# qdLMF/LightGlue-with-FlashAttentionV2-TensorRT

Hardware: AMD Instinct MI355X
Metric: attention-calls/sec & ms/call, 1×1024×1024 d=64 fp16; % MFMA peak (higher is better)
Workload: dtype fp16; 1 GPU; MHAHeadDim64 plugin enqueue, Q/K/V [1,4,1024,64] fp16 -> O fp16 (BASELINE configs[1]); K independent plugin enqueues per timed repetition; batch=1, heads=4, nq=1024, nkv=1024, head_dim=64, parallelism=replicas1, pairs=one pair stream per GPU, no collective

## Files before the change

lightglue-with-flashattentionv2-tensorrt_amd/csrc/lightglue_ffn.hip:

```cpp
#include <stdlib.h>

#include <atomic>
#include <cstdlib>

#include "lightglue_device.h"

namespace {

#ifdef LG_LN_STAMPS
__device__ unsigned long long g_ln_stamps[256 * 8 * 8];
#define LN_SEG(k)                                                                                    \
    do {                                                                                             \
        unsigned long long t_;                                                                       \
        asm volatile("s_waitcnt lgkmcnt(0)\n\ts_memtime %0\n\ts_waitcnt lgkmcnt(0)" : "=s"(t_)::"memory"); \
        sg_[k] += t_ - last_;                                                                        \
        last_ = t_;                                                                                  \
    } while (0)
#else
#define LN_SEG(k) \
    do {          \
    } while (0)
#endif
constexpr int kLnN = 512;
template <int KS, int MT, int BK, int NST, int NWV = 8>
// ... 71 lines not shown
        for (int ks = 0; ks < KS; ++ks) {
            const int gs = t * KS + ks;
            if (ks == 0 && t == 0) LN_SEG(0);
            else LN_SEG(2);
            if (gs + NST - 2 > nsteps - 1) asm volatile("s_waitcnt vmcnt(0) lgkmcnt(0)" ::: "memory");
            else if (ks < NST - 1 && t > 0) asm volatile("s_waitcnt vmcnt(%0) lgkmcnt(0)" ::"n"((NST - 2) * D + SPW) : "memory");
            else asm volatile("s_waitcnt vmcnt(%0) lgkmcnt(0)" ::"n"((NST - 2) * D) : "memory");
            __builtin_amdgcn_s_barrier();
            LN_SEG(1);
            {
                char* const fb = smem + (st == 0 ? NST - 1 : st - 1) * SB;
                if (ks + NST - 1 < KS) tile_issue<true, BK, KS, NT, NWV>(cur, ks + NST - 1, fb, wave);
                else if (more) tile_issue<true, BK, KS, NT, NWV>(src_of(t + 1), ks + NST - 1 - KS, fb, wave);
            }
            const unsigned sb = (unsigned)(st * SB);
            st_last = st;
            st = st == NST - 1 ? 0 : st + 1;
#pragma unroll
            for (int s = 0; s < BK / 16; ++s) {
                const int u = 2 * s + hh;
                f16x8 wf[NB], af[2];
#pragma unroll
                for (int b = 0; b < NB; ++b) wf[b] = *(lds_f16x8*)(lds + sb + wro[b] + ((u ^ wsw[b]) << 4));
#pragma unroll
                for (int b = 0; b < 2; ++b) af[b] = *(lds_f16x8*)(lds + sb + aro[b] + ((u ^ asw[b]) << 4));
#pragma unroll
                for (int nb = 0; nb < NB; ++nb)
#pragma unroll
                    for (int mb = 0; mb < 2; ++mb)
                        acc[nb][mb] = __builtin_amdgcn_mfma_f32_32x32x16_f16(wf[nb], af[mb], acc[nb][mb], 0, 0, 0);
            }
        }

        LN_SEG(2);
        const int nw0 = wn * WTN;
        float rs[2];
#pragma unroll
        for (int mb = 0; mb < 2; ++mb) {
            float s = 0.f;
#pragma unroll
            for (int nb = 0; nb < NB; ++nb)
#pragma unroll
                for (int g = 0; g < 4; ++g) {
                    const u32x2 b4 = *(__attribute__((address_space(3))) u32x2*)(lds + kPar + (nw0 + 32 * nb + 8 * g + 4 * hh) * 2);
#pragma unroll
                    for (int u = 0; u < 4; ++u) {
                        const float a = acc[nb][mb][4 * g + u];
                        const float h = (u & 1) ? mixh<1>(a, b4[u >> 1]) : mixh<0>(a, b4[u >> 1]);
                        acc[nb][mb][4 * g + u] = h;
                        s += h;
                    }
                }
            rs[mb] = s + __shfl_xor(s, 32, 64);
        }
        if (hh == 0) {
#pragma unroll
            for (int mb = 0; mb < 2; ++mb) red[(wm * 64 + 32 * mb + r) * WN + wn] = rs[mb];
        }
        asm volatile("s_waitcnt lgkmcnt(0)" ::: "memory");
        __builtin_amdgcn_s_barrier();
        float mean[2];
#pragma unroll
        for (int mb = 0; mb < 2; ++mb) {
            mean[mb] = red_sum((wm * 64 + 32 * mb + r) * WN) * (1.f / kLnN);
            float q = 0.f;
#pragma unroll
            for (int nb = 0; nb < NB; ++nb)
#pragma unroll
                for (int e = 0; e < 16; ++e) {
                    const float d = acc[nb][mb][e] - mean[mb];
                    acc[nb][mb][e] = d;
                    q = __builtin_fmaf(d, d, q);
                }
            rs[mb] = q + __shfl_xor(q, 32, 64);
        }
        if (hh == 0) {
#pragma unroll
            for (int mb = 0; mb < 2; ++mb) red[MT * WN + (wm * 64 + 32 * mb + r) * WN + wn] = rs[mb];
        }
        asm volatile("s_waitcnt lgkmcnt(0)" ::: "memory");
        __builtin_amdgcn_s_barrier();
        LN_SEG(3);
        lds_char* const stg = lds + st_last * SB + wave * 4096;
#pragma unroll
        for (int mb = 0; mb < 2; ++mb) {
            const float rstd = __builtin_amdgcn_rsqf(red_sum(MT * WN + (wm * 64 + 32 * mb + r) * WN) * (1.f / kLnN) + eps);
#pragma unroll
            for (int np = 0; np < NP; ++np) {
#pragma unroll
                for (int nbl = 0; nbl < 2; ++nbl)
#pragma unroll
                    for (int g = 0; g < 4; ++g) {
                        const int n = nw0 + 64 * np + 32 * nbl + 8 * g + 4 * hh;
                        const u32x2 g4 = *(__attribute__((address_space(3))) u32x2*)(lds + kPar + NT * 2 + n * 2);
                        const u32x2 b4 = *(__attribute__((address_space(3))) u32x2*)(lds + kPar + 2 * NT * 2 + n * 2);
                        f16x4 o;
#pragma unroll
                        for (int u = 0; u < 4; u += 2) {
                            const f32x16& av = acc[2 * np + nbl][mb];
                            const f32x2 xr = f32x2{av[4 * g + u], av[4 * g + u + 1]} * rstd;
                            const f32x2 gl = gelu_as2(f32x2{mixf<0>(xr[0], g4[u >> 1], b4[u >> 1]), mixf<1>(xr[1], g4[u >> 1], b4[u >> 1])});
                            o[u] = (f16)gl[0];
                            o[u + 1] = (f16)gl[1];
                        }
                        *(__attribute__((address_space(3))) f16x4*)(stg + r * 128 + (((4 * nbl + g) ^ (r & 7)) << 4) + 8 * hh) = o;
                    }
                f16x8 o8[4];
#pragma unroll
                for (int i = 0; i < 4; ++i) {
                    const int rl = 8 * i + cr;
                    o8[i] = *(lds_f16x8*)(stg + rl * 128 + ((cc ^ (rl & 7)) << 4));
                }
#pragma unroll
                for (int i = 0; i < 4; ++i) {
                    const int row = min(m0 + wm * 64 + 32 * mb + 8 * i + cr, p.m - 1);
                    st_out(p.out[0] + (size_t)row * NT + nw0 + 64 * np + 8 * cc, o8[i]);
                }
            }
        }
        if (more) cur = src_of(t + 1);
    }
    asm volatile("s_waitcnt vmcnt(0)" ::: "memory");
    LN_SEG(4);
#ifdef LG_LN_STAMPS
    if (lane == 0) {
        unsigned long long* d = g_ln_stamps + ((size_t)blockIdx.x * 8 + wave) * 8;
        for (int k = 0; k < 5; ++k) d[k] = sg_[k];
        d[5] = last_ - t_entry_;
        d[6] = (unsigned long long)ntile_w;
    }
#endif
}


constexpr int kFfnOut = 256;

enum { E3_NONE = 0, E3_SPLIT2 = 1, E3_QKV = 2, E3_PLAIN = 3 };
struct Proj3 {
    const f16* b3;
    const f16* cosv;
    const f16* sinv;
    f16* out[6];
    int n_store;
};
#ifdef LG_FR_STAMPS
__device__ unsigned long long g_fr_stamps[256 * 8 * 8];
#define FR_SEG(k)                                                                                    \
    do {                                                                                             \
        unsigned long long t_;                                                                       \
        asm volatile("s_waitcnt lgkmcnt(0)\n\ts_memtime %0\n\ts_waitcnt lgkmcnt(0)" : "=s"(t_)::"memory"); \
        fr_[k] = t_ - fr_last_;                                                                      \
        fr_last_ = t_;                                                                               \
    } while (0)
#else
#define FR_SEG(k) \
    do {          \
    } while (0)
#endif
__device__ __forceinline__ void row_dev2(unsigned h2, float c, f32x2& q) {
    const f32x2 d = f32x2{mixn<0>(h2, 1.f, -c), mixn<1>(h2, 1.f, -c)};
    q = d * d + q;
}
struct RowStats {
    float mean, rstd;
};
__device__ __forceinline__ RowStats ln_merge(f32x4 sa, f32x4 sc, f32x4 qa, f32x4 qc, float eps) {
    const float mean = (((sa[0] + sa[1]) + (sa[2] + sa[3])) + ((sc[0] + sc[1]) + (sc[2] + sc[3]))) * (1.f / 512);
    const f32x4 da = sa * (1.f / 64) - mean, dc = sc * (1.f / 64) - mean;
    const f32x4 ba = da * da, bc = dc * dc;
    const float within = ((qa[0] + qa[1]) + (qa[2] + qa[3])) + ((qc[0] + qc[1]) + (qc[2] + qc[3]));
    const float between = ((ba[0] + ba[1]) + (ba[2] + ba[3])) + ((bc[0] + bc[1]) + (bc[2] + bc[3]));
    return {mean, __builtin_amdgcn_rsqf(fmaf(between, 64.f, within) * (1.f / 512) + eps)};
}
template <int MB, int D, int E3, int NB3>
__global__ __launch_bounds__(512, 1) void ffn_rows_kernel(LinArgs p, const f16* __restrict__ gamma,
                                                          const f16* __restrict__ beta, float eps,
                                                          const f16* __restrict__ wp, const f16* __restrict__ b2,
                                                          Proj3 q3) {
    constexpr int MT = 32 * MB;
    constexpr int K = 512, NO = kFfnOut;
    constexpr int kA = 0, kH = MT * K * 2;
    constexpr int kSP = 80;
    constexpr int kStg = MB == 1 ? 2 * kH : kH;
    constexpr int kPar = MB == 1 ? kStg + 8 * MT * kSP : 2 * kH;
    constexpr int kRed = kPar + (3 * K + NO) * 2;
    constexpr int NS1 = K / 16, NS = 2 * NS1;
    constexpr int NS3 = NO / 16;
    constexpr int NP = 96 + NB3 * NS3;
    constexpr int R = 2 * D;
    static_assert(D >= 1 && D <= NS1 && (MB == 1 || MB == 2) && (E3 == E3_NONE) == (NB3 == 0), "shape");
    static_assert(MB == 1 || 8 * MT * kSP <= kH, "staging over h");
    constexpr int kB3 = kRed + 2 * MT * 8 * 4;
    constexpr int kCS = kB3 + NB3 * 256 * 2;
    constexpr int kCSP = 144;
    constexpr int kEnd = kCS + (E3 == E3_QKV ? 2 * MT * kCSP : 0);
    static_assert(kEnd <= 160 * 1024, "LDS");
    __shared__ __attribute__((aligned(16))) char smem[kEnd];
    lds_char* const lds = (lds_char*)smem;
    const int tid = threadIdx.x, lane = tid & 63;
    const int wave = __builtin_amdgcn_readfirstlane(tid >> 6);
    const int r = lane & 31, hh = lane >> 5;
    const int m0 = blockIdx.x * MT;
#ifdef LG_FR_STAMPS
    unsigned long long fr_[6] = {0, 0, 0, 0, 0, 0}, fr_last_, fr_entry_;
    asm volatile("s_memtime %0\n\ts_waitcnt lgkmcnt(0)" : "=s"(fr_entry_)::"memory");
    fr_last_ = fr_entry_;
#endif

    constexpr bool AH = MB == 1;
    f16x8 av[AH ? 1 : 4 * MB], ax[2 * MB], ac[2 * MB];
    if constexpr (AH) {
#pragma unroll
        for (int i = 0; i < 2 * MB; ++i) {
            const int grow = min(m0 + 16 * i + 2 * wave + (lane >> 5), p.m - 1);
            ax[i] = *reinterpret_cast<const f16x8*>(p.a + (size_t)grow * (K / 2) + (lane & 31) * 8);
        }
#pragma unroll
        for (int i = 0; i < 2 * MB; ++i) {
            const int grow = min(m0 + 16 * i + 2 * wave + (lane >> 5), p.m - 1);
            const LinRow lr = lin_row(p, grow, (lane & 31) >> 3);
            ac[i] = *reinterpret_cast<const f16x8*>((lr.first ? p.ctx0 : p.ctx1) + lr.off + (lane & 7) * 8);
        }
    } else {
#pragma unroll
        for (int i = 0; i < 4 * MB; ++i) {
            const int grow = min(m0 + 8 * i + wave, p.m - 1);
            const f16* src;
            if (lane < 32) {
                src = p.a + (size_t)grow * (K / 2) + lane * 8;
            } else {
                const LinRow lr = lin_row(p, grow, (lane - 32) >> 3);
                src = (lr.first ? p.ctx0 : p.ctx1) + lr.off + ((lane - 32) & 7) * 8;
            }
            av[i] = *reinterpret_cast<const f16x8*>(src);
        }
    }
    f16x8 pv = {};
    if (tid < 224) {
        const f16* const pvs = tid < 64 ? p.bias : tid < 128 ? gamma : tid < 192 ? beta : b2;
        pv = *reinterpret_cast<const f16x8*>(pvs + (tid & 63) * 8);
    }

    constexpr int NV3 = NB3 * 256 * 2 / 16 + (E3 == E3_QKV ? 2 * MT * kD * 2 / 16 : 0);
    constexpr int NV3T = (NV3 + 511) / 512;
    f16x8 v3[NV3T > 0 ? NV3T : 1];
#pragma unroll
    for (int i = 0; i < NV3T; ++i) {
        const int u = i * 512 + tid;
        if (u < NB3 * 256 * 2 / 16) {
            v3[i] = *reinterpret_cast<const f16x8*>(q3.b3 + u * 8);
        } else if (u < NV3) {
            const int cu = u - NB3 * 256 * 2 / 16, t = cu / (MT * 8), rw = min(m0 + (cu % (MT * 8)) / 8, p.m - 1);
            v3[i] = *reinterpret_cast<const f16x8*>((t ? q3.sinv : q3.cosv) + (size_t)rw * kD + (cu % 8) * 8);
        }
    }

    asm volatile("s_barrier" ::: "memory");

    const __amdgpu_buffer_rsrc_t wrs = __builtin_amdgcn_make_buffer_rsrc(const_cast<f16*>(wp), (short)0, 8 * NP * 1024, 0x00020000);
    const unsigned wo = (unsigned)(wave * NP * 1024 + lane * 16);
    auto piece = [&](int i) { return __builtin_bit_cast(f16x8, __builtin_amdgcn_raw_buffer_load_b128(wrs, wo, i * 1024, 0)); };
    f16x8 q[R];
#pragma unroll
    for (int i = 0; i < R; ++i) {
        q[i] = piece(i);
        if (i & 1) __builtin_amdgcn_sched_barrier(0);
    }
    auto take = [&](int i) {
        const f16x8 w = q[i % R];
        if (i + R < NP) q[i % R] = piece(i + R);
        return w;
    };
    auto put_half = [&](const f16x8 (&hv)[2 * MB], int u0) {
#pragma unroll
        for (int i = 0; i < 2 * MB; ++i) {
            const int row = 16 * i + 2 * wave + (lane >> 5), u = u0 + (lane & 31);
            *(lds_f16x8*)(lds + kA + row * 1024 + ((u ^ (row & 15)) << 4)) = hv[i];
        }
    };
    if constexpr (AH) {
        put_half(ax, 0);
    } else {
#pragma unroll
        for (int i = 0; i < 4 * MB; ++i) {
            const int row = 8 * i + wave;
            *(lds_f16x8*)(lds + kA + row * 1024 + ((lane ^ (row & 15)) << 4)) = av[i];
        }
    }
    if (tid < 224) *(lds_f16x8*)(lds + kPar + tid * 16) = pv;
#pragma unroll
    for (int i = 0; i < NV3T; ++i)
        if (i * 512 + tid < NB3 * 256 * 2 / 16) {
            *(lds_f16x8*)(lds + kB3 + (i * 512 + tid) * 16) = v3[i];
        } else if (i * 512 + tid < NV3) {
            const int cu = i * 512 + tid - NB3 * 256 * 2 / 16;
            *(lds_f16x8*)(lds + kCS + (cu / 8) * kCSP + (cu % 8) * 16) = v3[i];
        }
    asm volatile("s_waitcnt lgkmcnt(0)" ::: "memory");
    __builtin_amdgcn_s_barrier();
    FR_SEG(0);

    struct BF {
        f16x8 v[MB];
    };
    auto bfrag = [&](int base, int s) {
        BF f;
#pragma unroll
        for (int mb = 0; mb < MB; ++mb) {
// ... 109 lines not shown
        asm volatile("s_waitcnt lgkmcnt(0)" ::: "memory");
        __builtin_amdgcn_s_barrier();
    }

    lds_char* const stg = lds + kStg + wave * (MT * kSP);
#pragma unroll
    for (int mb = 0; mb < MB; ++mb)
#pragma unroll
        for (int g = 0; g < 4; ++g) {
            const int c = 32 * wave + 8 * g + 4 * hh;
            const f16x4 b4 = *(__attribute__((address_space(3))) f16x4*)(lds + kPar + 3 * K * 2 + c * 2);
            const f16x4 v = f16x4{lin_val(o2[mb][4 * g], b4[0]), lin_val(o2[mb][4 * g + 1], b4[1]),
                                  lin_val(o2[mb][4 * g + 2], b4[2]), lin_val(o2[mb][4 * g + 3], b4[3])};
            *(__attribute__((address_space(3))) f16x4*)(stg + (32 * mb + r) * kSP + (8 * g + 4 * hh) * 2) = v;
        }
    asm volatile("s_waitcnt lgkmcnt(0)" ::: "memory");
    f16x8 xo[MB][2];
#pragma unroll
    for (int mb = 0; mb < MB; ++mb) {
        const int rr = 32 * mb + (lane >> 1), half = lane & 1;
#pragma unroll
        for (int e2 = 0; e2 < 2; ++e2) {
            f16x8 v = *(lds_f16x8*)(stg + rr * kSP + half * 32 + e2 * 16);
            const f16x8 xr = *(lds_f16x8*)(lds + kA + rr * 1024 + (((4 * wave + 2 * half + e2) ^ (rr & 15)) << 4));
#pragma unroll
            for (int e = 0; e < 8; ++e) v[e] = res_add(v[e], xr[e]);
            xo[mb][e2] = v;
            if (m0 + rr < p.m) *reinterpret_cast<f16x8*>(p.out[0] + (size_t)(m0 + rr) * NO + 32 * wave + 16 * half + 8 * e2) = v;
        }
    }
#ifdef LG_FR_STAMPS
    asm volatile("s_waitcnt vmcnt(0)" ::: "memory");
    FR_SEG(4);
#endif
    if constexpr (E3 != E3_NONE) {
        asm volatile("s_waitcnt lgkmcnt(0)" ::: "memory");
        __builtin_amdgcn_s_barrier();
#pragma unroll
        for (int mb = 0; mb < MB; ++mb) {
            const int rr = 32 * mb + (lane >> 1), half = lane & 1;
#pragma unroll
            for (int e2 = 0; e2 < 2; ++e2)
                *(lds_f16x8*)(lds + kA + rr * 512 + (((4 * wave + 2 * half + e2) ^ (rr & 15)) << 4)) = xo[mb][e2];
        }
        asm volatile("s_waitcnt lgkmcnt(0)" ::: "memory");
        __builtin_amdgcn_s_barrier();
        auto xfrag = [&](int s) {
            BF f;
#pragma unroll
            for (int mb = 0; mb < MB; ++mb) {
                const int row = 32 * mb + r;
                f.v[mb] = *(lds_f16x8*)(lds + kA + row * 512 + (((2 * s + hh) ^ (row & 15)) << 4));
            }
            return f;
        };
        f32x16 a3[NB3][MB] = {};
        BF xf = xfrag(0);
#pragma unroll
        for (int j = 0; j < NS3; ++j) {
            f16x8 w3[NB3];
#pragma unroll
            for (int b = 0; b < NB3; ++b) w3[b] = take(96 + NB3 * j + b);
            const BF xn = j + 1 < NS3 ? xfrag(j + 1) : xf;
#pragma unroll
            for (int b = 0; b < NB3; ++b)
#pragma unroll
                for (int mb = 0; mb < MB; ++mb) a3[b][mb] = __builtin_amdgcn_mfma_f32_32x32x16_f16(w3[b], xf.v[mb], a3[b][mb], 0, 0, 0);
            xf = xn;
            __builtin_amdgcn_sched_barrier(0);
        }
#pragma unroll
        for (int b = 0; b < NB3; ++b) {
            const int cb = 32 * (NB3 * wave + b);
#pragma unroll
            for (int mb = 0; mb < MB; ++mb)
#pragma unroll
                for (int g = 0; g < 4; ++g) {
                    const int c = cb + 8 * g + 4 * hh;
                    const f16x4 b4 = *(__attribute__((address_space(3))) f16x4*)(lds + kB3 + c * 2);
                    f16x4 v = f16x4{lin_val(a3[b][mb][4 * g], b4[0]), lin_val(a3[b][mb][4 * g + 1], b4[1]),
                                    lin_val(a3[b][mb][4 * g + 2], b4[2]), lin_val(a3[b][mb][4 * g + 3], b4[3])};
                    if constexpr (E3 == E3_QKV) {
                        if (cb < 2 * NO) {
                            const int rw = 32 * mb + r;
                            const f16x4 cc = *(__attribute__((address_space(3))) f16x4*)(lds + kCS + rw * kCSP + (c % kD) * 2);
                            const f16x4 ss = *(__attribute__((address_space(3))) f16x4*)(lds + kCS + (MT + rw) * kCSP + (c % kD) * 2);
#pragma unroll
                            for (int t = 0; t < 4; t += 2) rot_pair(v, t, cc[t], ss[t], cc[t + 1], ss[t + 1]);
                        }
                    }
                    *(__attribute__((address_space(3))) f16x4*)(stg + (32 * mb + r) * kSP + (8 * g + 4 * hh) * 2) = v;
                }
            asm volatile("s_waitcnt lgkmcnt(0)" ::: "memory");
#pragma unroll
            for (int mb = 0; mb < MB; ++mb) {
                const int rr = 32 * mb + (lane >> 1), half = lane & 1;
                const f16x8 v0 = *(lds_f16x8*)(stg + rr * kSP + half * 32);
                const f16x8 v1 = *(lds_f16x8*)(stg + rr * kSP + half * 32 + 16);
                const int row = m0 + rr;
                if (row < p.m) {
                    f16* dst;
                    if constexpr (E3 == E3_PLAIN) {
                        dst = cb < q3.n_store ? q3.out[0] + (size_t)row * q3.n_store + cb + 16 * half : nullptr;
                    } else {
                        const int part = cb / NO, h = (cb % NO) / kD;
                        const LinRow lr = lin_row(p, row, h);
                        dst = q3.out[E3 == E3_QKV ? (lr.first ? 0 : 3) + part : (lr.first ? 0 : 1) + 2 * part] + lr.off +
                              cb % kD + 16 * half;
                    }
                    if (dst) {
                        *reinterpret_cast<f16x8*>(dst) = v0;
                        *reinterpret_cast<f16x8*>(dst + 8) = v1;
                    }
                }
            }
            asm volatile("s_waitcnt lgkmcnt(0)" ::: "memory");
        }
    }
#ifdef LG_FR_STAMPS
    asm volatile("s_waitcnt vmcnt(0)" ::: "memory");
    FR_SEG(5);
    if (lane == 0 && blockIdx.x < 256) {
        unsigned long long* d = g_fr_stamps + ((size_t)blockIdx.x * 8 + wave) * 8;
        for (int k = 0; k < 5; ++k) d[k] = fr_[k];
        d[5] = fr_last_ - fr_entry_;
        d[6] = fr_entry_;
        d[7] = fr_[5];
    }
#endif
}

template <int D, int E3, int NB3, int SP = 1>
__global__ __launch_bounds__(512, 1) void ffn_rows16_kernel(LinArgs p, const f16* __restrict__ gamma,
                                                            const f16* __restrict__ beta, float eps,
                                                            const f16* __restrict__ wp, const f16* __restrict__ b2,
                                                            Proj3 q3) {
    constexpr int MT = 16, K = 512, NO = kFfnOut;
    constexpr int NP = 96 + NB3 * 16;
    constexpr int R = 2 * D;
    constexpr int NB = 2 * NB3;
    constexpr int NBP = NB / (SP > 1 ? SP : 1);
    constexpr int NPS = 96 + 8 * NBP;
    constexpr int U3 = 32 * NB3;
    constexpr int kA = 0;
    constexpr int kH = kA + MT * 1024;
    constexpr int kX = kH + MT * 1024;
    constexpr int kS3 = kX + MT * 512;
    constexpr int kPar = kS3 + MT * U3 * 16;
    constexpr int kRed = kPar + (3 * K + NO) * 2;
    constexpr int kB3 = kRed + 2 * MT * 8 * 4;
    constexpr int kCS = kB3 + NB3 * 256 * 2;
    constexpr int kCSP = 144;
    constexpr int kEnd = kCS + (E3 == E3_QKV ? 2 * MT * kCSP : 0);
    static_assert(D >= 1 && D <= 16 && (E3 == E3_NONE) == (NB3 == 0) && kEnd <= 160 * 1024, "shape");
    static_assert(SP == 1 || (E3 != E3_NONE && NB % SP == 0), "parts");
    __shared__ __attribute__((aligned(16))) char smem[kEnd];
    lds_char* const lds = (lds_char*)smem;
    const int tid = threadIdx.x, lane = tid & 63;
    const int wave = __builtin_amdgcn_readfirstlane(tid >> 6);
    const int r = lane & 15, q = lane >> 4;
    const int part = SP > 1 ? (int)blockIdx.x % SP : 0;
    const int m0 = (SP > 1 ? (int)blockIdx.x / SP : (int)blockIdx.x) * MT;
#ifdef LG_FR_STAMPS
    unsigned long long fr_[7] = {0, 0, 0, 0, 0, 0, 0}, fr_last_, fr_entry_;
    asm volatile("s_memtime %0\n\ts_waitcnt lgkmcnt(0)" : "=s"(fr_entry_)::"memory");
    fr_last_ = fr_entry_;
#endif
    auto tile_unit = [](int row, int u) { return row * 1024 + ((u ^ (row & 15)) << 4); };
    auto x_unit = [](int row, int u) { return row * 512 + ((u ^ (row & 15)) << 4); };

    f16x8 ax, ac;
    {
        const int grow = min(m0 + (tid >> 5), p.m - 1);
        ax = *reinterpret_cast<const f16x8*>(p.a + (size_t)grow * (K / 2) + (tid & 31) * 8);
        const LinRow lr = lin_row(p, grow, (tid & 31) >> 3);
        ac = *reinterpret_cast<const f16x8*>((lr.first ? p.ctx0 : p.ctx1) + lr.off + (tid & 7) * 8);
    }
    f16x8 pv = {};
    if (tid < 224) {
        const f16* const pvs = tid < 64 ? p.bias : tid < 128 ? gamma : tid < 192 ? beta : b2;
        pv = *reinterpret_cast<const f16x8*>(pvs + (tid & 63) * 8);
    }
    constexpr int NVB = NB3 * 256 * 2 / 16;
    constexpr int NV3 = NVB + (E3 == E3_QKV ? 2 * MT * 8 : 0);
    static_assert(NV3 <= 512, "phase 3 vectors");
    f16x8 v3 = {};
    if (tid < NV3) {
        if (tid < NVB) {
            v3 = *reinterpret_cast<const f16x8*>(q3.b3 + tid * 8);
        } else {
            const int cu = tid - NVB, t = cu / (MT * 8), rw = min(m0 + (cu % (MT * 8)) / 8, p.m - 1);
            v3 = *reinterpret_cast<const f16x8*>((t ? q3.sinv : q3.cosv) + (size_t)rw * kD + (cu % 8) * 8);
        }
    }
    asm volatile("s_barrier" ::: "memory");

    const __amdgpu_buffer_rsrc_t wrs = __builtin_amdgcn_make_buffer_rsrc(const_cast<f16*>(wp), (short)0, 8 * NP * 1024, 0x00020000);
    const unsigned wo = (unsigned)(wave * NP * 1024 + lane * 16);
    const int p3off = __builtin_amdgcn_readfirstlane(part * NBP * 1024);
    auto piece = [&](int i) {
        const int so = i < 96 ? i * 1024 : (96 + NB * ((i - 96) / NBP) + (i - 96) % NBP) * 1024 + p3off;
        return __builtin_bit_cast(f16x8, __builtin_amdgcn_raw_buffer_load_b128(wrs, wo, so, 0));
    };
    f16x8 w_[R];
#pragma unroll
    for (int i = 0; i < R; ++i) {
        w_[i] = piece(i);
        if (i & 1) __builtin_amdgcn_sched_barrier(0);
    }
    auto take = [&](int i) {
        const f16x8 w = w_[i % R];
        if (i + R < NPS) w_[i % R] = piece(i + R);
        return w;
    };
    *(lds_f16x8*)(lds + kA + tile_unit(tid >> 5, tid & 31)) = ax;
    if (tid < 224) *(lds_f16x8*)(lds + kPar + tid * 16) = pv;
    if (tid < NVB) {
        *(lds_f16x8*)(lds + kB3 + tid * 16) = v3;
    } else if (tid < NV3) {
        const int cu = tid - NVB;
        *(lds_f16x8*)(lds + kCS + (cu / 8) * kCSP + (cu % 8) * 16) = v3;
    }
    asm volatile("s_waitcnt lgkmcnt(0)" ::: "memory");
    __builtin_amdgcn_s_barrier();
    FR_SEG(0);

    f32x4 acc[4] = {};
    f16x8 bf = *(lds_f16x8*)(lds + kA + tile_unit(r, q));
#pragma unroll
    for (int s = 0; s < 16; ++s) {
        f16x8 w4[4];
#pragma unroll
        for (int b = 0; b < 4; ++b) w4[b] = take(4 * s + b);
        if (s + 1 == 8) {
            *(lds_f16x8*)(lds + kA + tile_unit(tid >> 5, 32 + (tid & 31))) = ac;
            asm volatile("s_waitcnt lgkmcnt(0)" ::: "memory");
            __builtin_amdgcn_s_barrier();
        }
        const f16x8 bn = s + 1 < 16 ? *(lds_f16x8*)(lds + kA + tile_unit(r, 4 * (s + 1) + q)) : bf;
#pragma unroll
        for (int b = 0; b < 4; ++b) acc[b] = __builtin_amdgcn_mfma_f32_16x16x32_f16(w4[b], bf, acc[b], 0, 0, 0);
        bf = bn;
        __builtin_amdgcn_sched_barrier(0);
    }
    FR_SEG(1);

    float* const red = (float*)(void*)(smem + kRed);
    float s1 = 0.f;
    f32x2 sd = {0.f, 0.f};
    unsigned hp[4][2];
#pragma unroll
    for (int b = 0; b < 4; ++b) {
        const u32x2 b4 = *(__attribute__((address_space(3))) u32x2*)(lds + kPar + (64 * wave + 16 * b + 4 * q) * 2);
#pragma unroll
        for (int u = 0; u < 2; ++u) {
            hp[b][u] = mixh2(acc[b][2 * u], acc[b][2 * u + 1], b4[u]);
            row_sum2(hp[b][u], s1);
        }
    }
    auto xsum = [](float x) {
        const auto a = __builtin_amdgcn_permlane16_swap(__float_as_uint(x), __float_as_uint(x), false, false);
        const float y = __uint_as_float(a[0]) + __uint_as_float(a[1]);
        const auto c = __builtin_amdgcn_permlane32_swap(__float_as_uint(y), __float_as_uint(y), false, false);
        return __uint_as_float(c[0]) + __uint_as_float(c[1]);
    };
    s1 = xsum(s1);
#pragma unroll
    for (int b = 0; b < 4; ++b)
#pragma unroll
        for (int u = 0; u < 2; ++u) row_dev2(hp[b][u], s1 * (1.f / 64), sd);
    const float s2 = xsum(sd[0] + sd[1]);
    if (q == 0) {
        red[r * 8 + wave] = s1;
        red[MT * 8 + r * 8 + wave] = s2;
    }
    asm volatile("s_waitcnt lgkmcnt(0)" ::: "memory");
    __builtin_amdgcn_s_barrier();
    auto row_stats = [&](int row) {
        auto part = [&](int i) { return *(__attribute__((address_space(3))) f32x4*)(lds + kRed + (i + row * 8) * 4); };
        return ln_merge(part(0), part(4), part(MT * 8), part(MT * 8 + 4), eps);
    };
    {
        const RowStats st = row_stats(r);
        const float rstd = st.rstd, nmr = -st.mean * rstd;
#pragma unroll
        for (int b = 0; b < 4; ++b) {
            const int n = 64 * wave + 16 * b + 4 * q;
            const u32x2 g4 = *(__attribute__((address_space(3))) u32x2*)(lds + kPar + K * 2 + n * 2);
            const u32x2 be4 = *(__attribute__((address_space(3))) u32x2*)(lds + kPar + 2 * K * 2 + n * 2);
            f16x4 o;
#pragma unroll
            for (int u = 0; u < 2; ++u) {
                const float x0 = mixn<0>(hp[b][u], rstd, nmr), x1 = mixn<1>(hp[b][u], rstd, nmr);
                const f32x2 gl = gelu_as2(f32x2{mixf<0>(x0, g4[u], be4[u]), mixf<1>(x1, g4[u], be4[u])});
                o[2 * u] = (f16)gl[0];
                o[2 * u + 1] = (f16)gl[1];
            }
            *(__attribute__((address_space(3))) f16x4*)(lds + kH + tile_unit(r, n >> 3) + 8 * (q & 1)) = o;
        }
    }
    asm volatile("s_waitcnt lgkmcnt(0)" ::: "memory");
    __builtin_amdgcn_s_barrier();
    FR_SEG(2);

    f32x4 o2[2] = {};
    f16x8 hf = *(lds_f16x8*)(lds + kH + tile_unit(r, q));
#pragma unroll
    for (int s = 0; s < 16; ++s) {
        const f16x8 wa = take(64 + 2 * s), wb = take(64 + 2 * s + 1);
        const f16x8 hn = s + 1 < 16 ? *(lds_f16x8*)(lds + kH + tile_unit(r, 4 * (s + 1) + q)) : hf;
        o2[0] = __builtin_amdgcn_mfma_f32_16x16x32_f16(wa, hf, o2[0], 0, 0, 0);
        o2[1] = __builtin_amdgcn_mfma_f32_16x16x32_f16(wb, hf, o2[1], 0, 0, 0);
        hf = hn;
        __builtin_amdgcn_sched_barrier(0);
    }
    FR_SEG(3);
#pragma unroll
    for (int b = 0; b < 2; ++b) {
        const int c = 32 * wave + 16 * b + 4 * q;
        const f16x4 b4 = *(__attribute__((address_space(3))) f16x4*)(lds + kPar + 3 * K * 2 + c * 2);
        const f16x4 v = f16x4{lin_val(o2[b][0], b4[0]), lin_val(o2[b][1], b4[1]), lin_val(o2[b][2], b4[2]),
                              lin_val(o2[b][3], b4[3])};
        *(__attribute__((address_space(3))) f16x4*)(lds + kX + x_unit(r, c >> 3) + 8 * (q & 1)) = v;
    }
    asm volatile("s_waitcnt lgkmcnt(0)" ::: "memory");
    __builtin_amdgcn_s_barrier();
    {
        const int row = tid >> 5, u = tid & 31;
        f16x8 v = *(lds_f16x8*)(lds + kX + x_unit(row, u));
        const f16x8 xr = *(lds_f16x8*)(lds + kA + tile_unit(row, u));
#pragma unroll
        for (int e = 0; e < 8; ++e) v[e] = res_add(v[e], xr[e]);
        if (part == 0 && m0 + row < p.m) *reinterpret_cast<f16x8*>(p.out[0] + (size_t)(m0 + row) * NO + 8 * u) = v;
        if constexpr (E3 != E3_NONE) *(lds_f16x8*)(lds + kX + x_unit(row, u)) = v;
    }
#ifdef LG_FR_STAMPS
    asm volatile("s_waitcnt vmcnt(0)" ::: "memory");
    FR_SEG(4);
#endif
    if constexpr (E3 != E3_NONE) {
        asm volatile("s_waitcnt lgkmcnt(0)" ::: "memory");
        __builtin_amdgcn_s_barrier();
        f16x4 rc[E3 == E3_QKV ? NBP : 1], rs[E3 == E3_QKV ? NBP : 1];
        if constexpr (E3 == E3_QKV) {
#pragma unroll
            for (int b = 0; b < NBP; ++b) {
                const int d = (16 * (NB * wave + part * NBP + b) + 4 * q) % kD;
                rc[b] = *(__attribute__((address_space(3))) f16x4*)(lds + kCS + r * kCSP + d * 2);
                rs[b] = *(__attribute__((address_space(3))) f16x4*)(lds + kCS + (MT + r) * kCSP + d * 2);
            }
        }
        f32x4 a3[NBP] = {};
        f16x8 xf = *(lds_f16x8*)(lds + kX + x_unit(r, q));
#pragma unroll
        for (int s = 0; s < 8; ++s) {
            f16x8 w3[NBP];
#pragma unroll
            for (int b = 0; b < NBP; ++b) w3[b] = take(96 + NBP * s + b);
            const f16x8 xn = s + 1 < 8 ? *(lds_f16x8*)(lds + kX + x_unit(r, 4 * (s + 1) + q)) : xf;
#pragma unroll
            for (int b = 0; b < NBP; ++b) a3[b] = __builtin_amdgcn_mfma_f32_16x16x32_f16(w3[b], xf, a3[b], 0, 0, 0);
            xf = xn;
            __builtin_amdgcn_sched_barrier(0);
        }
        FR_SEG(5);
#pragma unroll
        for (int b = 0; b < NBP; ++b) {
            const int c = 16 * (NB * wave + part * NBP + b) + 4 * q;
            const f16x4 b4 = *(__attribute__((address_space(3))) f16x4*)(lds + kB3 + c * 2);
            f16x4 v = f16x4{lin_val(a3[b][0], b4[0]), lin_val(a3[b][1], b4[1]), lin_val(a3[b][2], b4[2]),
                            lin_val(a3[b][3], b4[3])};
            constexpr bool ROT = E3 == E3_QKV;
            if constexpr (ROT) {
                if (c < 2 * NO) {
#pragma unroll
                    for (int t = 0; t < 4; t += 2) rot_pair(v, t, rc[b][t], rs[b][t], rc[b][t + 1], rs[b][t + 1]);
                }
            }
            *(__attribute__((address_space(3))) f16x4*)(lds + kS3 + r * (U3 * 16) + (((c >> 3) ^ r) << 4) + 8 * (q & 1)) = v;
        }
        asm volatile("s_waitcnt lgkmcnt(0)" ::: "memory");
        __builtin_amdgcn_s_barrier();
        {
            const int row = tid >> 5, t = tid & 31, grow = m0 + row;
            if (grow < p.m) {
                if constexpr (E3 == E3_PLAIN) {
#pragma unroll
                    for (int j = 0; j < U3 / 32; ++j) {
                        const int u = t + 32 * j;
                        if (SP > 1 && ((8 * u) % (16 * NB)) / (16 * NBP) != part) continue;
                        if (8 * u < q3.n_store)
                            *reinterpret_cast<f16x8*>(q3.out[0] + (size_t)grow * q3.n_store + 8 * u) =
                                *(lds_f16x8*)(lds + kS3 + row * (U3 * 16) + ((u ^ row) << 4));
                    }
                } else {
                    const LinRow lr = lin_row(p, grow, t >> 3);
                    const size_t off = lr.off + (8 * t) % kD;
#pragma unroll
                    for (int j = 0; j < U3 / 32; ++j) {
                        const int u = t + 32 * j;
                        if (SP > 1 && ((8 * u) % (16 * NB)) / (16 * NBP) != part) continue;
                        const f16x8 v = *(lds_f16x8*)(lds + kS3 + row * (U3 * 16) + ((u ^ row) << 4));
                        f16* const dst = q3.out[E3 == E3_QKV ? (lr.first ? 0 : 3) + j : (lr.first ? 0 : 1) + 2 * j] + off;
                        *reinterpret_cast<f16x8*>(dst) = v;
                    }
                }
            }
        }
    }
#ifdef LG_FR_STAMPS
    asm volatile("s_waitcnt vmcnt(0)" ::: "memory");
    FR_SEG(6);
    if (lane == 0 && blockIdx.x < 256) {
        unsigned long long* d = g_fr_stamps + ((size_t)blockIdx.x * 8 + wave) * 8;
        for (int i = 0; i < 5; ++i) d[i] = fr_[i];
        d[5] = fr_last_ - fr_entry_;
        d[6] = fr_[6];
        d[7] = fr_[5];
    }
#endif
}

__global__ __launch_bounds__(256) void ffn_pack_kernel(const f16* __restrict__ w1, const f16* __restrict__ w2,
                                                       const f16* __restrict__ w3, int nb3, int form, f16* packed) {
    const int np = 96 + 16 * nb3;
    const int f = blockIdx.x * 256 + threadIdx.x;
    if (f >= 8 * np * 64) return;
    const int w = f / (np * 64), i = (f % (np * 64)) / 64, l = f % 64;
    const f16* src;
    if (form == 0) {
        const int r = l % 32, hh = l / 32;
        if (i < 64) src = w1 + (size_t)(64 * w + 32 * (i & 1) + r) * 512 + 16 * (i >> 1) + 8 * hh;
        else if (i < 96) src = w2 + (size_t)(32 * w + r) * 512 + 16 * (i - 64) + 8 * hh;
        else {
            const int j = (i - 96) / nb3, b = (i - 96) % nb3;
            src = w3 + (size_t)(32 * (nb3 * w + b) + r) * 256 + 16 * j + 8 * hh;
        }
    } else {
        const int r = l % 16, q = l / 16;
        if (i < 64) src = w1 + (size_t)(64 * w + 16 * (i & 3) + r) * 512 + 32 * (i >> 2) + 8 * q;
        else if (i < 96) src = w2 + (size_t)(32 * w + 16 * ((i - 64) & 1) + r) * 512 + 32 * ((i - 64) >> 1) + 8 * q;
        else {
            const int j = (i - 96) / (2 * nb3), b = (i - 96) % (2 * nb3);
            src = w3 + (size_t)(16 * (2 * nb3 * w + b) + r) * 256 + 32 * j + 8 * q;
        }
    }
    *reinterpret_cast<f16x8*>(packed + (size_t)f * 8) = *reinterpret_cast<const f16x8*>(src);
}

std::atomic<int> g_ln_fused{1};
}

extern "C" {

int32_t lg_linear_set_ln_fused(int32_t on) { return g_ln_fused.exchange(on == 2 ? 2 : on ? 1 : 0); }

int32_t lg_linear_cat_ln_gelu(const void* x, const void* ctx0, const void* ctx1, int32_t heads, int32_t n0, int32_t n1,
                              int32_t pairs, const void* w, const void* bias, const void* gamma, const void* beta,
                              float eps, void* out, hipStream_t stream) {
    const int k = 2 * heads * kD, m = pairs * (n0 + n1), n = k;
    if (heads <= 0 || n0 < 0 || n1 < 0 || pairs < 0 || !shape_ok(m, n, k) || !x || !w || !bias || !gamma || !beta ||
        !out || !aligned16(x) || (n0 && !aligned16(ctx0)) || (n1 && !aligned16(ctx1)) || !aligned16(w) ||
        !aligned8(bias) || !aligned8(out) || !(eps >= 0.f))
        return bad("lg_linear_cat_ln_gelu");
    if (m == 0) return MHA_HD64_STATUS_SUCCESS;
    const int lnf = g_ln_fused.load();
    const bool big = m >= 128 * kTileGrid;
    const bool fused = lnf && n == kLnN && (lnf == 2 || big || m >= 64 * kTileGrid) && aligned16(bias) && aligned16(gamma) &&
                       aligned16(beta) && aligned16(out) && lightglue::wide_mode() != 0;
    if (!fused) {
        const int32_t st = lg_linear_cat(x, ctx0, ctx1, heads, n0, n1, pairs, w, bias, n, out, stream);
        if (st != MHA_HD64_STATUS_SUCCESS) return st;
        return lg_layernorm_gelu(MHA_HD64_DT_HALF, out, gamma, beta, m, n, eps, out, stream);
    }
    LinArgs p = gather_args(x, ctx0, ctx1, w, bias, out, heads, n0, n1, pairs, n, k);
    p.mtiles = big ? (m + 127) / 128 : (m + 63) / 64;
    p.total = p.mtiles;
    const int grid = p.total < kTileGrid ? p.total : kTileGrid;
    if (big)
        hipLaunchKernelGGL((linear_ln_kernel<512 / 32, 128, 32, 3>), dim3(grid), dim3(512), 0, stream, p,
                           (const f16*)gamma, (const f16*)beta, eps);
    else
        hipLaunchKernelGGL((linear_ln_kernel<512 / 64, 64, 64, 2>), dim3(grid), dim3(512), 0, stream, p,
                           (const f16*)gamma, (const f16*)beta, eps);
    return launched("lg_linear_cat_ln_gelu");
}

}

namespace {

std::atomic<int> g_ffn_fused{1};
}
extern "C" int32_t lg_linear_set_ffn_fused(int32_t mode) { return g_ffn_fused.exchange(mode >= 0 && mode <= 3 ? mode : 1); }

namespace {
constexpr int kFrDepth = 12;
int ffn_split_parts(int tiles) {
    static const int env = [] {
        const char* e = std::getenv("LG_FFN_SPLIT");
        return e ? std::atoi(e) : -1;
    }();
    if (env == 0) return 1;
    return (env == 2 ? 2 * tiles <= kTileGrid : tiles <= 64) ? 2 : 1;
}
template <int E3, int NB3>
void launch_ffn_rows(const LinArgs& p, const f16* gamma, const f16* beta, float eps, const f16* wp, const f16* b2,
                     const Proj3& q3, hipStream_t stream) {
    const int mode = g_ffn_fused.load();
    if (mode == 3 || (mode != 2 && p.m <= 16 * kTileGrid)) {
        const f16* wp16 = wp + (size_t)8 * (96 + 16 * NB3) * 1024 / 2;
        const int tiles = (p.m + 15) / 16;
        if constexpr (E3 != E3_NONE) {
            const int sp = ffn_split_parts(tiles);
            if (sp == 2) {
                hipLaunchKernelGGL((ffn_rows16_kernel<kFrDepth, E3, NB3, 2>), dim3(2 * tiles), dim3(512), 0, stream, p,
                                   gamma, beta, eps, wp16, b2, q3);
                return;
            }
        }
        hipLaunchKernelGGL((ffn_rows16_kernel<kFrDepth, E3, NB3>), dim3(tiles), dim3(512), 0, stream, p, gamma, beta, eps,
                           wp16, b2, q3);
    } else if (p.m <= 32 * kTileGrid)
        hipLaunchKernelGGL((ffn_rows_kernel<1, kFrDepth, E3, NB3>), dim3((p.m + 31) / 32), dim3(512), 0, stream, p, gamma, beta,
                           eps, wp, b2, q3);
    else
        hipLaunchKernelGGL((ffn_rows_kernel<2, kFrDepth, E3, NB3>), dim3((p.m + 63) / 64), dim3(512), 0, stream, p, gamma, beta,
                           eps, wp, b2, q3);
}
}

extern "C" {

int32_t lg_linear_cat_ffn(const void* x, const void* ctx0, const void* ctx1, int32_t heads, int32_t n0, int32_t n1,
                          int32_t pairs, const void* w1, const void* b1, const void* gamma, const void* beta, float eps,
                          const void* w2, const void* b2, const void* w_packed, void* h, void* out, hipStream_t stream) {
    const int d = heads * kD, k = 2 * d, m = pairs * (n0 + n1);
    if (heads <= 0 || n0 < 0 || n1 < 0 || pairs < 0 || !shape_ok(m, k, k) || !x || !w1 || !b1 || !gamma || !beta || !w2 ||
        !b2 || !h || !out || out == x || !aligned16(x) || (n0 && !aligned16(ctx0)) || (n1 && !aligned16(ctx1)) ||
        !aligned16(w1) || !aligned16(w2) || !aligned8(b1) || !aligned8(b2) || !aligned16(h) || !aligned8(out) || !(eps >= 0.f) ||
        (w_packed && !aligned16(w_packed)))
        return bad("lg_linear_cat_ffn");
    if (m == 0) return MHA_HD64_STATUS_SUCCESS;
    const bool one = g_ffn_fused.load() != 0 && w_packed && k == kLnN && d == kFfnOut && aligned16(b1) && aligned16(gamma) &&
                     aligned16(beta) && aligned16(b2) && aligned16(out);
    if (!one) {
        const int32_t st = lg_linear_cat_ln_gelu(x, ctx0, ctx1, heads, n0, n1, pairs, w1, b1, gamma, beta, eps, h, stream);
        if (st != MHA_HD64_STATUS_SUCCESS) return st;
        return lg_linear(h, w2, b2, x, m, d, k, out, stream);
    }
    const LinArgs p = gather_args(x, ctx0, ctx1, w1, b1, out, heads, n0, n1, pairs, k, k);
    launch_ffn_rows<E3_NONE, 0>(p, (const f16*)gamma, (const f16*)beta, eps, (const f16*)w_packed, (const f16*)b2, Proj3{}, stream);
    return launched("lg_linear_cat_ffn");
}

size_t lg_ffn_packed_bytes(int32_t heads, int32_t n3) {
    return heads == 4 && (n3 == 0 || n3 == 512 || n3 == 768) ? (size_t)2 * 8 * (96 + n3 / 16) * 1024 : 0;
}

int32_t lg_ffn_pack(const void* w1, const void* w2, const void* w3, int32_t n3, int32_t heads, void* packed, hipStream_t stream) {
    if (!lg_ffn_packed_bytes(heads, n3) || !w1 || !w2 || !packed || !aligned16(w1) || !aligned16(w2) || !aligned16(packed) ||
        (n3 && (!w3 || !aligned16(w3))))
        return bad("lg_ffn_pack");
    const int nb3 = n3 / 256, frags = 8 * (96 + 16 * nb3) * 64;
    for (int form = 0; form < 2; ++form)
        hipLaunchKernelGGL(ffn_pack_kernel, dim3((frags + 255) / 256), dim3(256), 0, stream, (const f16*)w1, (const f16*)w2,
                           (const f16*)w3, nb3, form, (f16*)packed + (size_t)form * frags * 8);
    return launched("lg_ffn_pack");
}

int32_t lg_linear_cat_ffn_proj(const void* x, const void* ctx0, const void* ctx1, int32_t heads, int32_t n0, int32_t n1,
                               int32_t pairs, const void* b1, const void* gamma, const void* beta, float eps, const void* b2,
                               const void* w_packed, int32_t kind, const void* b3, const void* cosv, const void* sinv,
                               int32_t n_store, void* const* outs3, void* out, hipStream_t stream) {
    const int d = heads * kD, k = 2 * d, m = pairs * (n0 + n1);
    const int nouts = kind == LG_PROJ_SPLIT2 ? 4 : kind == LG_PROJ_QKV ? 6 : kind == LG_PROJ_PLAIN ? 1 : 0;
    bool ok = heads == 4 && n0 >= 0 && n1 >= 0 && pairs >= 0 && nouts && x && b1 && gamma && beta && b2 && w_packed && b3 && outs3 &&
              out && out != x && aligned16(x) && (!n0 || aligned16(ctx0)) && (!n1 || aligned16(ctx1)) && aligned16(b1) &&
              aligned16(gamma) && aligned16(beta) && aligned16(b2) && aligned16(w_packed) && aligned8(b3) && aligned16(out) &&
              eps >= 0.f && (kind != LG_PROJ_QKV || (cosv && sinv && aligned8(cosv) && aligned8(sinv))) &&
              (kind != LG_PROJ_PLAIN || (n_store > 0 && n_store <= 512 && n_store % 8 == 0)) &&
              (kind == LG_PROJ_PLAIN || (long long)m * heads * kD < (1LL << 31));
    for (int i = 0; ok && i < nouts; ++i) ok = outs3[i] && aligned16(outs3[i]);
    if (!ok) return bad("lg_linear_cat_ffn_proj");
    if (m == 0) return MHA_HD64_STATUS_SUCCESS;
    const LinArgs p = gather_args(x, ctx0, ctx1, nullptr, b1, out, heads, n0, n1, pairs, k, k);
    Proj3 q3{};
    q3.b3 = (const f16*)b3, q3.cosv = (const f16*)cosv, q3.sinv = (const f16*)sinv, q3.n_store = n_store;
    for (int i = 0; i < nouts; ++i) q3.out[i] = (f16*)outs3[i];
    const f16 *g = (const f16*)gamma, *be = (const f16*)beta, *wp = (const f16*)w_packed, *bb2 = (const f16*)b2;
    if (kind == LG_PROJ_SPLIT2) launch_ffn_rows<E3_SPLIT2, 2>(p, g, be, eps, wp, bb2, q3, stream);
    else if (kind == LG_PROJ_QKV) launch_ffn_rows<E3_QKV, 3>(p, g, be, eps, wp, bb2, q3, stream);
    else launch_ffn_rows<E3_PLAIN, 2>(p, g, be, eps, wp, bb2, q3, stream);
    return launched("lg_linear_cat_ffn_proj");
}

#ifdef LG_LN_STAMPS
int32_t lg_diag_ln_stamps(void* host_dst) {
    return hipMemcpyFromSymbol(host_dst, HIP_SYMBOL(g_ln_stamps), sizeof(g_ln_stamps)) == hipSuccess ? 0 : 1;
}
#endif
#ifdef LG_FR_STAMPS
int32_t lg_diag_fr_stamps(void* host_dst) {
    return hipMemcpyFromSymbol(host_dst, HIP_SYMBOL(g_fr_stamps), sizeof(g_fr_stamps)) == hipSuccess ? 0 : 1;
}
#endif

}
```

Before: 210,400 calls/s.

## Defer FFN side-input loads into weight prefetch and hoist LN parameter reads

The FFN rows kernel now issues the context, bias/gamma/beta and rope/bias3 global loads after the first weight pieces, inside the weight-prefetch loop. Their LDS stores move to the mid-GEMM barrier, and the LN parameters are read from LDS before the LayerNorm stage. Output and cos/sin pointers are pinned in scalar registers, and the default split-parts heuristic changes to use the grid-based rule. The intent is to get the weight stream started sooner and shorten the LN critical path, at the cost of more live registers. Optional sub-stage timestamp instrumentation is also added.

```diff
diff --git a/lightglue-with-flashattentionv2-tensorrt_amd/csrc/lightglue_ffn.hip b/lightglue-with-flashattentionv2-tensorrt_amd/csrc/lightglue_ffn.hip
--- a/lightglue-with-flashattentionv2-tensorrt_amd/csrc/lightglue_ffn.hip
+++ b/lightglue-with-flashattentionv2-tensorrt_amd/csrc/lightglue_ffn.hip
@@ -247,8 +247,22 @@
         fr_[k] = t_ - fr_last_;                                                                      \
         fr_last_ = t_;                                                                               \
     } while (0)
+__device__ unsigned long long g_fr_substamps[256 * 8 * 8];
+#define FR_SUB(k)                                                                                    \
+    do {                                                                                             \
+        unsigned long long t_;                                                                       \
+        asm volatile("s_waitcnt lgkmcnt(0)\n\ts_memtime %0\n\ts_waitcnt lgkmcnt(0)" : "=s"(t_)::"memory"); \
+        fs_[k] = t_ - fr_last_;                                                                      \
+    } while (0)
+#define FR_DEP(x) asm volatile("" ::"v"(x))
 #else
 #define FR_SEG(k) \
+    do {          \
+    } while (0)
+#define FR_SUB(k) \
+    do {          \
+    } while (0)
+#define FR_DEP(x) \
     do {          \
     } while (0)
 #endif
@@ -664,7 +678,7 @@
     constexpr int kCS = kB3 + NB3 * 256 * 2;
     constexpr int kCSP = 144;
     constexpr int kEnd = kCS + (E3 == E3_QKV ? 2 * MT * kCSP : 0);
-    static_assert(D >= 1 && D <= 16 && (E3 == E3_NONE) == (NB3 == 0) && kEnd <= 160 * 1024, "shape");
+    static_assert(D >= 4 && D <= 16 && (E3 == E3_NONE) == (NB3 == 0) && kEnd <= 160 * 1024, "shape");
     static_assert(SP == 1 || (E3 != E3_NONE && NB % SP == 0), "parts");
     __shared__ __attribute__((aligned(16))) char smem[kEnd];
     lds_char* const lds = (lds_char*)smem;
@@ -674,7 +688,7 @@
     const int part = SP > 1 ? (int)blockIdx.x % SP : 0;
     const int m0 = (SP > 1 ? (int)blockIdx.x / SP : (int)blockIdx.x) * MT;
 #ifdef LG_FR_STAMPS
-    unsigned long long fr_[7] = {0, 0, 0, 0, 0, 0, 0}, fr_last_, fr_entry_;
+    unsigned long long fr_[7] = {0, 0, 0, 0, 0, 0, 0}, fs_[5] = {0, 0, 0, 0, 0}, fr_last_, fr_entry_;
     asm volatile("s_memtime %0\n\ts_waitcnt lgkmcnt(0)" : "=s"(fr_entry_)::"memory");
     fr_last_ = fr_entry_;
 #endif
@@ -682,29 +696,44 @@
     auto x_unit = [](int row, int u) { return row * 512 + ((u ^ (row & 15)) << 4); };
 
     f16x8 ax, ac;
-    {
-        const int grow = min(m0 + (tid >> 5), p.m - 1);
-        ax = *reinterpret_cast<const f16x8*>(p.a + (size_t)grow * (K / 2) + (tid & 31) * 8);
-        const LinRow lr = lin_row(p, grow, (tid & 31) >> 3);
-        ac = *reinterpret_cast<const f16x8*>((lr.first ? p.ctx0 : p.ctx1) + lr.off + (tid & 7) * 8);
-    }
-    f16x8 pv = {};
-    if (tid < 224) {
-        const f16* const pvs = tid < 64 ? p.bias : tid < 128 ? gamma : tid < 192 ? beta : b2;
-        pv = *reinterpret_cast<const f16x8*>(pvs + (tid & 63) * 8);
-    }
+    const int grow_a = min(m0 + (tid >> 5), p.m - 1);
+    ax = *reinterpret_cast<const f16x8*>(p.a + (size_t)grow_a * (K / 2) + (tid & 31) * 8);
+    const LinRow lr_a = lin_row(p, grow_a, (tid & 31) >> 3);
+    const size_t off_a = lr_a.off + (tid & 7) * 8;
+    const f16* const ac_src = (lr_a.first ? p.ctx0 : p.ctx1) + off_a;
     constexpr int NVB = NB3 * 256 * 2 / 16;
     constexpr int NV3 = NVB + (E3 == E3_QKV ? 2 * MT * 8 : 0);
     static_assert(NV3 <= 512, "phase 3 vectors");
-    f16x8 v3 = {};
-    if (tid < NV3) {
-        if (tid < NVB) {
-            v3 = *reinterpret_cast<const f16x8*>(q3.b3 + tid * 8);
-        } else {
-            const int cu = tid - NVB, t = cu / (MT * 8), rw = min(m0 + (cu % (MT * 8)) / 8, p.m - 1);
-            v3 = *reinterpret_cast<const f16x8*>((t ? q3.sinv : q3.cosv) + (size_t)rw * kD + (cu % 8) * 8);
-        }
-    }
+    asm volatile("" ::"s"(eps), "s"(p.out[0]), "s"(p.bias), "s"(gamma), "s"(beta), "s"(b2), "s"(q3.b3));
+    typedef __attribute__((address_space(1))) f16x8 glb_f16x8;
+    unsigned long long o3[6] = {}, cos3 = 0, sin3 = 0;
+    if constexpr (E3 != E3_NONE) {
+#pragma unroll
+        for (int j = 0; j < (E3 == E3_QKV ? 6 : E3 == E3_SPLIT2 ? 4 : 1); ++j) {
+            o3[j] = (unsigned long long)q3.out[j];
+            asm volatile("" : "+s"(o3[j]));
+        }
+        if constexpr (E3 == E3_QKV) {
+            cos3 = (unsigned long long)q3.cosv, sin3 = (unsigned long long)q3.sinv;
+            asm volatile("" : "+s"(cos3), "+s"(sin3));
+        }
+    }
+    f16x8 pv = {}, v3 = {};
+    auto load_rest = [&]() {
+        ac = *reinterpret_cast<const f16x8*>(ac_src);
+        if (tid < 224) {
+            const f16* const pvs = tid < 64 ? p.bias : tid < 128 ? gamma : tid < 192 ? beta : b2;
+            pv = *reinterpret_cast<const f16x8*>(pvs + (tid & 63) * 8);
+        }
+        if (tid < NV3) {
+            if (tid < NVB) {
+                v3 = *reinterpret_cast<const f16x8*>(q3.b3 + tid * 8);
+            } else {
+                const int cu = tid - NVB, t = cu / (MT * 8), rw = min(m0 + (cu % (MT * 8)) / 8, p.m - 1);
+                v3 = *(const glb_f16x8*)((t ? sin3 : cos3) + ((size_t)rw * kD + (cu % 8) * 8) * 2);
+            }
+        }
+    };
     asm volatile("s_barrier" ::: "memory");
 
     const __amdgpu_buffer_rsrc_t wrs = __builtin_amdgcn_make_buffer_rsrc(const_cast<f16*>(wp), (short)0, 8 * NP * 1024, 0x00020000);
@@ -719,6 +748,10 @@
     for (int i = 0; i < R; ++i) {
         w_[i] = piece(i);
         if (i & 1) __builtin_amdgcn_sched_barrier(0);
+        if (i == 7) {
+            load_rest();
+            __builtin_amdgcn_sched_barrier(0);
+        }
     }
     auto take = [&](int i) {
         const f16x8 w = w_[i % R];
@@ -726,19 +759,13 @@
         return w;
     };
     *(lds_f16x8*)(lds + kA + tile_unit(tid >> 5, tid & 31)) = ax;
-    if (tid < 224) *(lds_f16x8*)(lds + kPar + tid * 16) = pv;
-    if (tid < NVB) {
-        *(lds_f16x8*)(lds + kB3 + tid * 16) = v3;
-    } else if (tid < NV3) {
-        const int cu = tid - NVB;
-        *(lds_f16x8*)(lds + kCS + (cu / 8) * kCSP + (cu % 8) * 16) = v3;
-    }
     asm volatile("s_waitcnt lgkmcnt(0)" ::: "memory");
     __builtin_amdgcn_s_barrier();
     FR_SEG(0);
 
     f32x4 acc[4] = {};
     f16x8 bf = *(lds_f16x8*)(lds + kA + tile_unit(r, q));
+    u32x2 b1v[4], g4[4], be4[4];
 #pragma unroll
     for (int s = 0; s < 16; ++s) {
         f16x8 w4[4];
@@ -746,8 +773,24 @@
         for (int b = 0; b < 4; ++b) w4[b] = take(4 * s + b);
         if (s + 1 == 8) {
             *(lds_f16x8*)(lds + kA + tile_unit(tid >> 5, 32 + (tid & 31))) = ac;
+            if (tid < 224) *(lds_f16x8*)(lds + kPar + tid * 16) = pv;
+            if (tid < NVB) {
+                *(lds_f16x8*)(lds + kB3 + tid * 16) = v3;
+            } else if (tid < NV3) {
+                const int cu = tid - NVB;
+                *(lds_f16x8*)(lds + kCS + (cu / 8) * kCSP + (cu % 8) * 16) = v3;
+            }
             asm volatile("s_waitcnt lgkmcnt(0)" ::: "memory");
             __builtin_amdgcn_s_barrier();
+        }
+        if (s + 1 == 16) {
+#pragma unroll
+            for (int b = 0; b < 4; ++b) {
+                const int n = 64 * wave + 16 * b + 4 * q;
+                b1v[b] = *(__attribute__((address_space(3))) u32x2*)(lds + kPar + n * 2);
+                g4[b] = *(__attribute__((address_space(3))) u32x2*)(lds + kPar + K * 2 + n * 2);
+                be4[b] = *(__attribute__((address_space(3))) u32x2*)(lds + kPar + 2 * K * 2 + n * 2);
+            }
         }
         const f16x8 bn = s + 1 < 16 ? *(lds_f16x8*)(lds + kA + tile_unit(r, 4 * (s + 1) + q)) : bf;
 #pragma unroll
@@ -763,10 +806,9 @@
     unsigned hp[4][2];
 #pragma unroll
     for (int b = 0; b < 4; ++b) {
-        const u32x2 b4 = *(__attribute__((address_space(3))) u32x2*)(lds + kPar + (64 * wave + 16 * b + 4 * q) * 2);
 #pragma unroll
         for (int u = 0; u < 2; ++u) {
-            hp[b][u] = mixh2(acc[b][2 * u], acc[b][2 * u + 1], b4[u]);
+            hp[b][u] = mixh2(acc[b][2 * u], acc[b][2 * u + 1], b1v[b][u]);
             row_sum2(hp[b][u], s1);
         }
     }
@@ -788,6 +830,7 @@
     }
     asm volatile("s_waitcnt lgkmcnt(0)" ::: "memory");
     __builtin_amdgcn_s_barrier();
+    FR_SUB(0);
     auto row_stats = [&](int row) {
         auto part = [&](int i) { return *(__attribute__((address_space(3))) f32x4*)(lds + kRed + (i + row * 8) * 4); };
         return ln_merge(part(0), part(4), part(MT * 8), part(MT * 8 + 4), eps);
@@ -795,22 +838,23 @@
     {
         const RowStats st = row_stats(r);
         const float rstd = st.rstd, nmr = -st.mean * rstd;
+        FR_DEP(nmr);
+        FR_SUB(1);
 #pragma unroll
         for (int b = 0; b < 4; ++b) {
             const int n = 64 * wave + 16 * b + 4 * q;
-            const u32x2 g4 = *(__attribute__((address_space(3))) u32x2*)(lds + kPar + K * 2 + n * 2);
-            const u32x2 be4 = *(__attribute__((address_space(3))) u32x2*)(lds + kPar + 2 * K * 2 + n * 2);
             f16x4 o;
 #pragma unroll
             for (int u = 0; u < 2; ++u) {
                 const float x0 = mixn<0>(hp[b][u], rstd, nmr), x1 = mixn<1>(hp[b][u], rstd, nmr);
-                const f32x2 gl = gelu_as2(f32x2{mixf<0>(x0, g4[u], be4[u]), mixf<1>(x1, g4[u], be4[u])});
+                const f32x2 gl = gelu_as2(f32x2{mixf<0>(x0, g4[b][u], be4[b][u]), mixf<1>(x1, g4[b][u], be4[b][u])});
                 o[2 * u] = (f16)gl[0];
                 o[2 * u + 1] = (f16)gl[1];
             }
             *(__attribute__((address_space(3))) f16x4*)(lds + kH + tile_unit(r, n >> 3) + 8 * (q & 1)) = o;
         }
     }
+    FR_SUB(2);
     asm volatile("s_waitcnt lgkmcnt(0)" ::: "memory");
     __builtin_amdgcn_s_barrier();
     FR_SEG(2);
@@ -893,6 +937,7 @@
         }
         asm volatile("s_waitcnt lgkmcnt(0)" ::: "memory");
         __builtin_amdgcn_s_barrier();
+        FR_SUB(3);
         {
             const int row = tid >> 5, t = tid & 31, grow = m0 + row;
             if (grow < p.m) {
@@ -902,25 +947,24 @@
                         const int u = t + 32 * j;
                         if (SP > 1 && ((8 * u) % (16 * NB)) / (16 * NBP) != part) continue;
                         if (8 * u < q3.n_store)
-                            *reinterpret_cast<f16x8*>(q3.out[0] + (size_t)grow * q3.n_store + 8 * u) =
+                            *(glb_f16x8*)(o3[0] + ((size_t)grow * q3.n_store + 8 * u) * 2) =
                                 *(lds_f16x8*)(lds + kS3 + row * (U3 * 16) + ((u ^ row) << 4));
                     }
                 } else {
-                    const LinRow lr = lin_row(p, grow, t >> 3);
-                    const size_t off = lr.off + (8 * t) % kD;
 #pragma unroll
                     for (int j = 0; j < U3 / 32; ++j) {
                         const int u = t + 32 * j;
                         if (SP > 1 && ((8 * u) % (16 * NB)) / (16 * NBP) != part) continue;
                         const f16x8 v = *(lds_f16x8*)(lds + kS3 + row * (U3 * 16) + ((u ^ row) << 4));
-                        f16* const dst = q3.out[E3 == E3_QKV ? (lr.first ? 0 : 3) + j : (lr.first ? 0 : 1) + 2 * j] + off;
-                        *reinterpret_cast<f16x8*>(dst) = v;
+                        const unsigned long long d0 = o3[E3 == E3_QKV ? j : 2 * j], d1 = o3[E3 == E3_QKV ? 3 + j : 1 + 2 * j];
+                        *(glb_f16x8*)((lr_a.first ? d0 : d1) + off_a * 2) = v;
                     }
                 }
             }
         }
     }
 #ifdef LG_FR_STAMPS
+    FR_SUB(4);
     asm volatile("s_waitcnt vmcnt(0)" ::: "memory");
     FR_SEG(6);
     if (lane == 0 && blockIdx.x < 256) {
@@ -929,6 +973,8 @@
         d[5] = fr_last_ - fr_entry_;
         d[6] = fr_[6];
         d[7] = fr_[5];
+        unsigned long long* e = g_fr_substamps + ((size_t)blockIdx.x * 8 + wave) * 8;
+        for (int i = 0; i < 5; ++i) e[i] = fs_[i];
     }
 #endif
 }
@@ -1014,7 +1060,7 @@
         return e ? std::atoi(e) : -1;
     }();
     if (env == 0) return 1;
-    return (env == 2 ? 2 * tiles <= kTileGrid : tiles <= 64) ? 2 : 1;
+    return (env == 1 ? tiles <= 64 : 2 * tiles <= kTileGrid) ? 2 : 1;
 }
 template <int E3, int NB3>
 void launch_ffn_rows(const LinArgs& p, const f16* gamma, const f16* beta, float eps, const f16* wp, const f16* b2,
@@ -1116,6 +1162,9 @@
 int32_t lg_diag_fr_stamps(void* host_dst) {
     return hipMemcpyFromSymbol(host_dst, HIP_SYMBOL(g_fr_stamps), sizeof(g_fr_stamps)) == hipSuccess ? 0 : 1;
 }
+int32_t lg_diag_fr_substamps(void* host_dst) {
+    return hipMemcpyFromSymbol(host_dst, HIP_SYMBOL(g_fr_substamps), sizeof(g_fr_substamps)) == hipSuccess ? 0 : 1;
+}
 #endif
 
 }
```

Result: no change. 210,300 calls/s (median of 2 runs) (-0.0%).
